# anadodik/sdmm-mitsuba

Measured on AMD Instinct MI355X. Metric: EM samples/sec (NxK resp) at K=128, N=2^20, higher is better.
Workload: dtype f32; 1 GPU; responsibility E-step, synthetic 5D sample batch (configs[1]); K=128, N=1048576, global_batch=1048576, samples_per_gpu=1048576, parallelism=sample-sharded x1 (strong: N fixed), layout=SoA fp32 in, [N][K] fp32 out

## Files before the change

sdmm-mitsuba_amd/csrc/estep_split.hip:

```cpp
#include "sdmm_device.h"

namespace sdmm {

namespace {

typedef float f2 __attribute__((ext_vector_type(2)));
typedef float f4 __attribute__((ext_vector_type(4)));
typedef __bf16 bf8 __attribute__((ext_vector_type(8)));
typedef __bf16 bf2 __attribute__((ext_vector_type(2)));
typedef unsigned u4 __attribute__((ext_vector_type(4)));

template <bool B> struct Tag { static constexpr bool value = B; };

constexpr float kLog2Norm5S = -6.628740082514092f;

__device__ __forceinline__ f2 spl(float x) { return (f2)(x); }
__device__ __forceinline__ f2 pfma(f2 a, f2 b, f2 c) { return __builtin_elementwise_fma(a, b, c); }
__device__ __forceinline__ f2 pmul(f2 a, f2 b) { return a * b; }
__device__ __forceinline__ f2 padd(f2 a, f2 b) { return a + b; }

__device__ __forceinline__ unsigned pk(float lo, float hi) {
    const bf2 v = __builtin_convertvector(f2{lo, hi}, bf2);
    return __builtin_bit_cast(unsigned, v);
}
// ... 375 lines not shown
#pragma unroll
        for (int r = 0; r < R; ++r)
#pragma unroll
            for (int j = 0; j < 4; ++j) {
                pdf[r][j] = P3[j & 1] + D3[j >> 1] + (float)(16 * r + j);
                acc.x += pdf[r][j];
            }
#else
        {
            bf8 F[2][8];
            f4 dp[2];
            frags(0, F[0], dp[0]);
#pragma unroll
            for (int r = 0; r < R; ++r) {
                f4 D[8];
                forms(F[r & 1], Bs, Bd, D);
                __builtin_amdgcn_sched_barrier(0);
                pair_math(r, Tag<false>{}, D, dp[r & 1]);
                if (r + 1 < R) frags(r + 1, F[(r + 1) & 1], dp[(r + 1) & 1]);
                __builtin_amdgcn_sched_barrier(0);
            }
        }
#endif
        const bool odd = cbits > __builtin_bit_cast(uint32_t, -0.9999995f) || !((acc.x + acc.y) + (acc2.x + acc2.y) >= 0.0f);
        if (__builtin_amdgcn_ballot_w64(odd) != 0) {
            bf8 bd2 = Bd, bs2 = Bs;
            asm volatile("" : "+v"(bd2), "+v"(bs2));
            acc = f2{0.0f, 0.0f};
            acc2 = f2{0.0f, 0.0f};
#pragma unroll
            for (int r = 0; r < R; ++r) {
                bf8 F[8];
                f4 dp, D[8];
                frags(r, F, dp);
                forms(F, bs2, bd2, D);
                pair_math(r, Tag<true>{}, D, dp);
            }
        }
        float S = (acc.x + acc.y) + (acc2.x + acc2.y);
        S += __shfl_xor(S, 16);
        S += __shfl_xor(S, 32);
        const float S2 = dif ? fmaf(1.0f - kHeuristicWeight, S, kHeuristicWeight * hp) : S;
        const float inv = __builtin_amdgcn_rcpf(S2);
        const bool fin = __builtin_isfinite(inv) && !dzero;
        gsc_p = fin ? (dif ? inv * (1.0f - kHeuristicWeight) : inv) : 0.0f;
        const bool bad = __builtin_amdgcn_ballot_w64(!__builtin_isfinite(S)) != 0;
        full_p = (t + 16 <= s1) && (16 * R == K) && !bad;
        tp = t;
    }
    flush();
    wait_vm<0>();
}

#ifndef SDMM_SPLIT_R8_WPB
#define SDMM_SPLIT_R8_WPB 12
#define SDMM_SPLIT_R8_OCC 3
#endif
#define SDMM_SPLIT_CONFIGS(X) X(1, 4, 4) X(2, 4, 4) X(4, 4, 4) X(8, SDMM_SPLIT_R8_WPB, SDMM_SPLIT_R8_OCC)

static void split_cfg(int R, int , int* wpb, int* occ) {
    *wpb = 4;
    *occ = 4;
    if (R == 8) {
        *wpb = SDMM_SPLIT_R8_WPB;
        *occ = SDMM_SPLIT_R8_OCC;
    }
}

bool estep_resp_split_supported(int Kp) { return Kp % 16 == 0 && Kp / 16 <= 8 && (Kp / 16 & (Kp / 16 - 1)) == 0; }

hipError_t launch_estep_resp_split(int variant, const float* ep, int Kp, int K, const SamplesDev& s, int64_t n,
                                   int64_t resident_waves, float* resp, hipStream_t st) {
    if (!estep_resp_split_supported(Kp) || K > Kp || resident_waves <= 0) return hipErrorInvalidValue;
    const int R = Kp / 16;
    int wpb, occ;
    split_cfg(R, variant, &wpb, &occ);
    const int64_t tiles = (n + 15) / 16;
    const int64_t blocks = ((tiles < resident_waves ? tiles : resident_waves) + wpb - 1) / wpb;
    const int64_t waves = blocks * wpb;
#define X(RR, WW, OO)                                                                                          \
    if (R == RR && wpb == WW && occ == OO) {                                                                   \
        hipLaunchKernelGGL((estep_resp_split_kernel<RR, WW, OO>), dim3((unsigned)blocks), dim3(64 * WW), 0, st, ep, \
                           Kp, K, s, n, waves, resp);                                                          \
        return hipGetLastError();                                                                              \
    }
    SDMM_SPLIT_CONFIGS(X)
#undef X
    return hipErrorInvalidValue;
}

hipError_t estep_resp_split_occupancy(int variant, int Kp, int* waves_per_cu) {
    const int R = Kp / 16;
    int wpb, occ;
    split_cfg(R, variant, &wpb, &occ);
    int blocks = 0;
#define X(RR, WW, OO)                                                                                          \
    if (R == RR && wpb == WW && occ == OO) {                                                                   \
        hipError_t e = hipOccupancyMaxActiveBlocksPerMultiprocessor(                                           \
            &blocks, reinterpret_cast<const void*>(&estep_resp_split_kernel<RR, WW, OO>), 64 * WW, 0);         \
        *waves_per_cu = blocks * WW;                                                                           \
        return e;                                                                                              \
    }
    SDMM_SPLIT_CONFIGS(X)
#undef X
    return hipErrorInvalidValue;
}

const char* estep_resp_split_name(int variant, int Kp) {
    static thread_local char buf[64];
    int wpb, occ;
    split_cfg(Kp / 16, variant, &wpb, &occ);
    snprintf(buf, sizeof buf, "estep_resp_split_kernel<%d,%d,%d>", Kp / 16, wpb, occ);
    return buf;
}

}
```

sdmm-mitsuba_amd/csrc/sdmm_api.cpp:

```cpp
#include <hip/hip_runtime.h>
#include <rccl/rccl.h>

#include <cmath>
#include <cstdlib>
#include <cstdio>
#include <cstring>
#include <new>
#include <string>
#include <vector>
#include <algorithm>
#include <atomic>
#include <future>
#include <thread>
#include <mutex>

#include "../../include/sdmm_gpu.h"
#include "sdmm_device.h"
#include "render_device.h"
#include "host_xfer.h"

#pragma clang fp contract(off)

namespace sdmm {
hipError_t launch_estep_resp(int cpl, int lps, const float* ep, int Kp, int K, const SamplesDev& s,
// ... 356 lines not shown
        float cov[25] = {0};
        for (int i = 0; i < 5; ++i) cov[6 * i] = 1.0f;
        for (int i = 0; i < 3; ++i)
            for (int j = 0; j < 3; ++j)
                cov[5 * i + j] = (s[i] * s[j] * widthVarSqr + t[i] * t[j] * widthVarSqr) +
                                 n[i] * n[j] * depthVarSqr;
        const float dcov = (float)(2.0 * PI * (double)directionalInit);
        cov[18] = dcov; cov[24] = dcov; cov[19] = 0.0f; cov[23] = 0.0f;
        float bPrior[25] = {0};
        for (int i = 0; i < 5; ++i) bPrior[6 * i] = 1.0f;
        for (int i = 0; i < 3; ++i)
            for (int j = 0; j < 3; ++j)
                bPrior[5 * i + j] = s[i] * s[j] * 1e-4f + t[i] * t[j] * 1e-4f + n[i] * n[j] * 1e-4f;
        bPrior[18] = 1e-5f; bPrior[24] = 1e-5f;
        float theta = 0.0f;
        for (int ti = 0; ti < (int)nThetas; ++ti) {
            float rn = (float)(((double)rng.next_float() - 0.5) * 2e-1);
            theta = (float)((double)theta + (0.5 * PI / (double)(nThetas + 1.0f) + (double)rn));
            const float cosTheta = fl_cos(theta);
            const float sinTheta = std::sqrt(1.0f - cosTheta * cosTheta);
            float phi = 0.0f;
            for (int fi = 0; fi < (int)nPhis; ++fi) {
                rn = (float)(((double)rng.next_float() - 0.5) * 1e-1);
                phi = (float)((double)phi + (2.0 * PI / (double)nPhis + (double)rn));
                const float sinPhi = fl_sin(phi), cosPhi = fl_cos(phi);
                const float dl0 = sinTheta * cosPhi, dl1 = sinTheta * sinPhi, dl2 = cosTheta;
                float* mean = means + 6 * k;
                for (int i = 0; i < 3; ++i) mean[i] = p[i];
                for (int i = 0; i < 3; ++i) mean[3 + i] = (s[i] * dl0 + t[i] * dl1) + n[i] * dl2;
                std::memcpy(covs + 25 * k, cov, sizeof(cov));
                weights[k] = 1.0f / (float)K;
                std::memcpy(bpriors + 25 * k, bPrior, sizeof(bPrior));
                for (int i = 0; i < 3; ++i)
                    for (int j = 0; j < 3; ++j) bdepth[9 * k + 3 * i + j] = n[i] * n[j] * 1e-6f;
                ++k;
            }
        }
    }
}

}

struct Slab {
    void* p = nullptr;
    std::atomic<int> refs{0};
    hipStream_t st = nullptr;
};

struct sdmm_mix {
    int K = 0, Kp = 0, cpl = 1, lps = 64;
    int rcpl = 2, rlps = 64;
    int rtile = 0;
    int rvariant = 4;
    int stile = 0;
    int svariant = 0;
    int device = 0;
    int cus = 256;
    int resp_blocks = 2, stats_blocks = 2;
    int guide_cap = kGuideCapDefault;
    mutable int* guide_fb = nullptr;
    mutable int64_t guide_fb_cap = 0;
    mutable GuideSortScratch guide_sort{};
    mutable ProductScratch product_scratch{};
    int guide_order = 1;
    hipStream_t stream = nullptr;
    hipStream_t own_stream = nullptr;
    sdmm_em_params params{};
    float norm2 = 0, norm3 = 0, norm5 = 0;
    bool initialised = false;

    void* block = nullptr;
    struct Slab* slab = nullptr;
    CanonDev C{};
    EmStateDev S{};
    float* ep = nullptr;
    float* gp = nullptr;
    double* stats = nullptr;
    double* tmp_mean = nullptr;
    double* tmp_cov = nullptr;
    unsigned* mcount = nullptr;
    float* partials = nullptr;
    int partial_rows = 0;
    int pstride = 0;
    void* staging = nullptr;
    size_t staging_bytes = 0;
    void* batch_dev = nullptr;
    void* batch_host = nullptr;
    mutable void* it_dev = nullptr;
    mutable void* it_host = nullptr;
    mutable size_t it_cap = 0;
    size_t batch_bytes = 0;
    hipEvent_t batch_copied = nullptr;
    hipEvent_t batch_done = nullptr;
    double* shard_stats = nullptr;
    size_t shard_bytes = 0;
};

struct sdmm_comm {
    int rank = 0, nranks = 1, device = 0;
    ncclComm_t nccl = nullptr;
    sdmm_host_allreduce_f64 h_allreduce = nullptr;
    sdmm_host_broadcast h_broadcast = nullptr;
    void* user = nullptr;
    void* pinned = nullptr;
    size_t pinned_bytes = 0;
};
// ... 272 lines not shown
        m->gp = gp;
        m->stats = stats;
        m->tmp_mean = tmean;
        m->tmp_cov = tcov;
        m->mcount = mcount;
    }
    return (off + 255) / 256 * 256;
}

void constructor_scalars(const sdmm_mix* m, double* scal) {
    for (int i = 0; i < SC_COUNT; ++i) scal[i] = 0.0;
    scal[SC_NORM] = 1.0;
    scal[SC_ALPHA] = (double)m->params.alpha;
    scal[SC_NI] = (double)m->params.ni_prior_minus_one;
    scal[SC_DECP] = m->params.decrease_prior ? 1.0 : 0.0;
    scal[SC_CUT] = 32.0;
}

struct OccCache {
    int K = -1, kern = -1, resp = 0, stats = 0;
};

int create_impl(int K, const sdmm_em_params* params, int device, hipStream_t ordered, bool on_stream,
                sdmm_mix** out, void* ext_block) {
    if (!out) return fail(SDMM_E_INVALID, "out is NULL");
    *out = nullptr;
    int cpl, lps;
    if (K < 1 || choose_layout(K, cpl, lps)) return fail(SDMM_E_INVALID, "K must be in [1, 512]");
    sdmm_mix* m = new (std::nothrow) sdmm_mix();
    if (!m) return fail(SDMM_E_NOMEM, "out of host memory");
    m->K = K;
    m->cpl = cpl;
    m->lps = lps;
    m->Kp = cpl * lps;
    m->device = device;
    if (params) m->params = *params; else sdmm_em_params_default(&m->params);
    m->norm2 = norm_const(2);
    m->norm3 = norm_const(3);
    m->norm5 = norm_const(5);
    m->pstride = ((ST_FIELDS * m->Kp + 2 + 3) / 4) * 4;

    auto cleanup = [&](int code) { sdmm_destroy(m); return code; };
    if (hipSetDevice(device) != hipSuccess) return cleanup(fail(SDMM_E_HIP, "hipSetDevice failed"));
    (void)hipDeviceGetAttribute(&m->cus, hipDeviceAttributeMultiprocessorCount, device);
    if (m->cus <= 0) m->cus = 256;
    m->rcpl = cpl;
    m->rlps = lps;
    if (K > 64 && K <= 128) { m->rcpl = 4; m->rlps = 32; }
    {
        const char* ev = std::getenv("SDMM_RESP_KERNEL");
        const bool legacy = ev && std::strcmp(ev, "legacy") == 0;
        const bool mfma = ev && std::strcmp(ev, "mfma") == 0;
        const bool tile = ev && std::strcmp(ev, "tile") == 0;
        const bool split = ev && std::strcmp(ev, "split") == 0;
        if (K > 64 && K <= 128 && !legacy && !mfma) {
            m->rtile = 1;
            m->rcpl = 2;
            m->rlps = 64;
            if (!tile && estep_resp_split_supported(m->Kp)) m->rtile = 3;
        }
        if (mfma) m->rtile = 2;
        if (split && estep_resp_split_supported(m->Kp)) m->rtile = 3;
        if (K > 64 && K <= 128) m->stile = 1;
        if (K > 128 && K <= 512) m->stile = 2;
    }
    static thread_local OccCache occ[8];
    OccCache& oc = occ[(K * 7 + device) & 7];
    const int kern = ((m->rtile * 16 + m->rvariant) * 16 + m->stile) * 16 + m->svariant;
    if (oc.K == K * 64 + device && oc.kern == kern) {
        m->resp_blocks = oc.resp;
        m->stats_blocks = oc.stats;
    } else {
        int unused = 0;
        if (estep_occupancy(m->rcpl, m->rlps, m->Kp, &m->resp_blocks, &unused) != hipSuccess ||
            estep_occupancy(m->cpl, m->lps, m->Kp, &unused, &m->stats_blocks) != hipSuccess)
            return cleanup(fail(SDMM_E_HIP, "E-step occupancy query failed"));
        if (m->rtile == 2 && estep_resp_mfma_occupancy(m->rvariant, m->Kp, &m->resp_blocks) != hipSuccess)
            return cleanup(fail(SDMM_E_HIP, "E-step occupancy query failed"));
        if (m->rtile == 3) {
            int wpc = 0;
            if (estep_resp_split_occupancy(m->rvariant, m->Kp, &wpc) != hipSuccess)
                return cleanup(fail(SDMM_E_HIP, "E-step occupancy query failed"));
            m->resp_blocks = wpc;
        }
        if (m->rtile == 1 && estep_resp_tile_occupancy(m->rvariant, &m->resp_blocks) != hipSuccess)
            return cleanup(fail(SDMM_E_HIP, "E-step occupancy query failed"));
        if (m->stile && estep_stats_tile_occupancy(m->svariant, m->Kp, &m->stats_blocks) != hipSuccess)
            return cleanup(fail(SDMM_E_HIP, "E-step occupancy query failed"));
        oc.K = K * 64 + device;
        oc.kern = kern;
        oc.resp = m->resp_blocks;
        oc.stats = m->stats_blocks;
    }
    if (on_stream) {
        m->stream = ordered;
    } else {
        if (hipStreamCreateWithFlags(&m->own_stream, hipStreamNonBlocking) != hipSuccess)
            return cleanup(fail(SDMM_E_HIP, "hipStreamCreate failed"));
        m->stream = m->own_stream;
    }

    if (ext_block) {
        layout_block(m, (char*)ext_block);
        *out = m;
        return SDMM_OK;
    }
    const size_t total = layout_block(m, nullptr);
    if (hipMalloc(&m->block, total) != hipSuccess) return cleanup(fail(SDMM_E_HIP, "hipMalloc failed"));
    if (hipMemsetAsync(m->block, 0, total, m->stream) != hipSuccess)
        return cleanup(fail(SDMM_E_HIP, "hipMemsetAsync failed"));
    layout_block(m, (char*)m->block);
    const size_t Kc = (size_t)K;
    double* sc = m->S.scalars;
    float* bp = m->S.bPriors;
    float* bd = m->S.bDepth;
    double scal[SC_COUNT];
    constructor_scalars(m, scal);
    (void)Kc;
    const float eps = (float)m->params.epsilon;
    if (launch_init_state(K, scal, m->params.bprior, eps, sc, bp, bd, m->stream) != hipSuccess)
        return cleanup(fail(SDMM_E_HIP, "state init kernel launch failed"));
    if (launch_pack_all(K, m->Kp, m->C, m->ep, m->gp, m->norm5, m->stream) != hipSuccess)
        return cleanup(fail(SDMM_E_HIP, "pack kernel launch failed"));
    if (!on_stream && hipStreamSynchronize(m->stream) != hipSuccess)
        return cleanup(fail(SDMM_E_HIP, "hipStreamSynchronize failed"));
    *out = m;
    return SDMM_OK;
}

int create_many(int K, const sdmm_em_params* params, int device, hipStream_t st, int n, sdmm_mix** out) {
    if (n < 0 || (n > 0 && !out)) return fail(SDMM_E_INVALID, "invalid argument");
    for (int i = 0; i < n; ++i) out[i] = nullptr;
    if (n == 0) return SDMM_OK;
    if (hipSetDevice(device) != hipSuccess) return fail(SDMM_E_HIP, "hipSetDevice failed");
// ... 172 lines not shown
    if (n < 0 || (n > 0 && (!src || !dst))) return fail(SDMM_E_INVALID, "invalid argument");
    if (n == 0) return SDMM_OK;
    int r = check_same_kind(src, n);
    if (!r) r = check_same_kind(dst, n);
    if (r) return r;
    if (src[0]->K != dst[0]->K || src[0]->device != dst[0]->device)
        return fail(SDMM_E_INVALID, "sources and destinations must share K and device");
    HIP_TRY(hipSetDevice(dst[0]->device));
    const hipStream_t st = dst[0]->stream;
    for (int i = 1; i < n; ++i)
        if (dst[i]->stream != st) HIP_TRY(hipStreamSynchronize(dst[i]->stream));
    return copy_prefix_many(src, dst, n, st);
}

int sdmm_num_components(const sdmm_mix* m) { return m ? m->K : 0; }

int sdmm_set_guide_order(sdmm_mix* m, int coherent) {
    if (!m) return fail(SDMM_E_INVALID, "null handle");
    m->guide_order = coherent ? 1 : 0;
    return SDMM_OK;
}

int sdmm_set_guide_capacity(sdmm_mix* m, int cap) {
    if (!m) return fail(SDMM_E_INVALID, "null handle");
    if (cap < 0 || cap > kGuideCapMax) return fail(SDMM_E_INVALID, "guide capacity must be in [0, 64]");
    m->guide_cap = cap;
    return SDMM_OK;
}

int sdmm_guide_fallback_count(const sdmm_mix* m, int* count) {
    if (!m || !count) return fail(SDMM_E_INVALID, "invalid argument");
    *count = 0;
    if (!m->guide_fb) return SDMM_OK;
    HIP_TRY(hipSetDevice(m->device));
    HIP_TRY(hipMemcpyAsync(count, m->guide_fb, sizeof(int), hipMemcpyDeviceToHost, m->stream));
    HIP_TRY(hipStreamSynchronize(m->stream));
    return SDMM_OK;
}

int sdmm_layout(const sdmm_mix* m, int* resp_cpl, int* resp_lps, int* stats_cpl, int* stats_lps) {
    if (!m) return fail(SDMM_E_INVALID, "null handle");
    if (resp_cpl) *resp_cpl = m->rcpl;
    if (resp_lps) *resp_lps = m->rlps;
    if (stats_cpl) *stats_cpl = m->cpl;
    if (stats_lps) *stats_lps = m->lps;
    return SDMM_OK;
}

const char* sdmm_kernel_name(const sdmm_mix* m, int which) {
    if (!m) return "";
    static thread_local char buf[64];
    if (which == 0) {
        if (m->rtile == 3) {
            std::snprintf(buf, sizeof buf, "%s", estep_resp_split_name(m->rvariant, m->Kp));
            return buf;
        } else if (m->rtile == 2) {
            std::snprintf(buf, sizeof buf, "%s", estep_resp_mfma_name(m->rvariant, m->Kp));
            return buf;
        } else if (m->rtile) {
            std::snprintf(buf, sizeof buf, "%s", estep_resp_tile_name(m->rvariant));
            return buf;
        }
        std::snprintf(buf, sizeof buf, "estep_resp_kernel<%d,%d>", m->rcpl, m->rlps);
        return buf;
    }
    if (m->stile == 2)
        std::snprintf(buf, sizeof buf, "estep_stats_tile_kernel<%d,2,true>", m->Kp / 128);
    else if (m->stile)
        std::snprintf(buf, sizeof buf, "estep_stats_tile_kernel<4,%d>", m->svariant == 1 ? 3 : 2);
    else
        std::snprintf(buf, sizeof buf, "estep_stats_kernel<%d,%d>", m->cpl, m->lps);
    return buf;
}

int sdmm_set_stream(sdmm_mix* m, void* hip_stream) {
    if (!m) return fail(SDMM_E_INVALID, "handle is NULL");
    HIP_TRY(hipSetDevice(m->device));
    if ((hipStream_t)hip_stream != m->stream) HIP_TRY(hipStreamSynchronize(m->stream));
    m->stream = (hipStream_t)hip_stream;
    return SDMM_OK;
}

void* sdmm_get_stream(const sdmm_mix* m) { return m ? (void*)m->stream : nullptr; }

int sdmm_synchronize(sdmm_mix* m) {
    if (!m) return fail(SDMM_E_INVALID, "handle is NULL");
    HIP_TRY(hipSetDevice(m->device));
    HIP_TRY(hipStreamSynchronize(m->stream));
    return SDMM_OK;
}

int sdmm_hemisphere_init_host(const float* positions, const float* normals, int n_pos, float depth_prior,
                              float min_spatial_distance, uint64_t seed, float* weights, float* means,
                              float* covs, float* bpriors, float* bdepth) {
    if (!positions || !normals || n_pos <= 0 || !weights || !means || !covs || !bpriors || !bdepth)
        return fail(SDMM_E_INVALID, "invalid argument to sdmm_hemisphere_init_host");
    hemisphere_init(positions, normals, n_pos, depth_prior, min_spatial_distance, seed, weights, means,
                    covs, bpriors, bdepth);
    return SDMM_OK;
}

static int upload_and_set(sdmm_mix* m, const float* weights, const float* means, const float* covs) {
    const size_t K = (size_t)m->K;
    char* pin = nullptr;
    HIP_TRY(bounce_buf(8 * 31 * K + 4 * K, &pin));
    double* md = (double*)pin;
    double* cd = md + 6 * K;
// ... 606 lines not shown
    r = stage_host_samples(m0, s, &d);
    if (r) return r;
    r = sdmm_em_step_batched(mixes, n_mix, &d, seg, iterations);
    const hipError_t e = hipStreamSynchronize(m0->stream);
    if (r) return r;
    if (e != hipSuccess) return fail(SDMM_E_HIP, std::string("sdmm_em_step_batched_host: ") + hipGetErrorString(e));
    return SDMM_OK;
}

int sdmm_em_step_batched_host_iters(sdmm_mix* const* mixes, int n_mix, const sdmm_samples* s, const int64_t* seg,
                                    const int* iterations) {
    if (n_mix < 0 || (n_mix > 0 && (!mixes || !mixes[0] || !iterations))) return fail(SDMM_E_INVALID, "invalid argument");
    if (n_mix == 0) return SDMM_OK;
    int r = check_samples(s);
    if (r) return r;
    if (s->n == 0) return sdmm_em_step_batched_iters(mixes, n_mix, s, seg, iterations);
    sdmm_mix* m0 = mixes[0];
    HIP_TRY(hipSetDevice(m0->device));
    sdmm_samples d;
    r = stage_host_samples(m0, s, &d);
    if (r) return r;
    r = sdmm_em_step_batched_iters(mixes, n_mix, &d, seg, iterations);
    const hipError_t e = hipStreamSynchronize(m0->stream);
    if (r) return r;
    if (e != hipSuccess) return fail(SDMM_E_HIP, std::string("sdmm_em_step_batched_host: ") + hipGetErrorString(e));
    return SDMM_OK;
}

int sdmm_em_step_host(sdmm_mix* m, const sdmm_samples* s, int iterations) {
    if (!m) return fail(SDMM_E_INVALID, "handle is NULL");
    HIP_TRY(hipSetDevice(m->device));
    int r = check_samples(s);
    if (r) return r;
    if (s->n == 0) return SDMM_OK;
    if (!m->initialised) return fail(SDMM_E_STATE, "mixture not initialised");
    sdmm_samples d;
    r = stage_host_samples(m, s, &d);
    if (r) return r;
    r = sdmm_em_step(m, &d, iterations);
    const hipError_t e = hipStreamSynchronize(m->stream);
    if (r) return r;
    if (e != hipSuccess) return fail(SDMM_E_HIP, std::string("sdmm_em_step_host: ") + hipGetErrorString(e));
    return SDMM_OK;
}

int sdmm_responsibilities(sdmm_mix* m, const sdmm_samples* s, float* resp) {
    if (!m || !resp) return fail(SDMM_E_INVALID, "invalid argument");
    if (!m->initialised) return fail(SDMM_E_STATE, "mixture not initialised");
    HIP_TRY(hipSetDevice(m->device));
    int r = check_samples(s);
    if (r) return r;
    if (s->n == 0) return SDMM_OK;
    if (m->rtile == 3) {
        const int64_t resident = (int64_t)m->cus * (m->resp_blocks > 0 ? m->resp_blocks : 1);
        HIP_TRY(launch_estep_resp_split(m->rvariant, m->ep, m->Kp, m->K, to_dev(s), s->n, resident, resp, m->stream));
        return SDMM_OK;
    }
    if (m->rtile == 2) {
        const int64_t resident = (int64_t)m->cus * 4 * (m->resp_blocks > 0 ? m->resp_blocks : 1);
        int64_t chunk = (s->n + 3 * resident - 1) / (3 * resident);
        chunk = ((chunk + 15) / 16) * 16;
        if (chunk < 64) chunk = 64;
        HIP_TRY(launch_estep_resp_mfma(m->rvariant, m->ep, m->Kp, m->K, to_dev(s), s->n, chunk, resp, m->stream));
        return SDMM_OK;
    }
    if (m->rtile) {
        const int64_t resident = (int64_t)m->cus * 4 * (m->resp_blocks > 0 ? m->resp_blocks : 1);
        int64_t chunk = (s->n + 3 * resident - 1) / (3 * resident);
        chunk = ((chunk + 63) / 64) * 64;
        if (chunk < 64) chunk = 64;
        HIP_TRY(launch_estep_resp_tile(m->rvariant, m->ep, m->Kp, m->K, to_dev(s), s->n, chunk, resp, m->stream));
        return SDMM_OK;
    }
    const Split sp = split_for(m, s->n, m->rlps, m->resp_blocks);
    HIP_TRY(launch_estep_resp(m->rcpl, m->rlps, m->ep, m->Kp, m->K, to_dev(s), s->n, sp.chunk, resp,
                              m->stream));
    return SDMM_OK;
}

int sdmm_guide_batch(const sdmm_mix* m, int64_t nq, const float* const c[3], const float* const u[3],
                     float* const d[3], float* pdf, int32_t* comp) {
    if (!m || !c || !u || !d || !pdf || !comp) return fail(SDMM_E_INVALID, "invalid argument");
    if (!m->initialised) return fail(SDMM_E_STATE, "mixture not initialised");
    HIP_TRY(hipSetDevice(m->device));
    if (nq <= 0) return SDMM_OK;
    int r = ensure_guide_scratch(m, nq);
    if (r) return r;
    HIP_TRY(launch_guide(m->gp, m->Kp, m->K, nq, c, u, nullptr, d, pdf, comp, m->norm2, m->norm3,
                         m->guide_cap, m->guide_fb, m->guide_fb + 1, m->cus, m->stream, guide_order(m, nq),
                         (int*)m->guide_sort.keys[0]));
    return SDMM_OK;
}

int sdmm_pdf_batch(const sdmm_mix* m, int64_t nq, const float* const c[3], const float* const d[3],
                   float* pdf) {
    if (!m || !c || !d || !pdf) return fail(SDMM_E_INVALID, "invalid argument");
    if (!m->initialised) return fail(SDMM_E_STATE, "mixture not initialised");
    HIP_TRY(hipSetDevice(m->device));
    if (nq <= 0) return SDMM_OK;
    int r = ensure_guide_scratch(m, nq);
    if (r) return r;
    HIP_TRY(launch_guide(m->gp, m->Kp, m->K, nq, c, nullptr, d, nullptr, pdf, nullptr, m->norm2, m->norm3,
                         m->guide_cap, m->guide_fb, m->guide_fb + 1, m->cus, m->stream, guide_order(m, nq),
                         (int*)m->guide_sort.keys[0]));
    return SDMM_OK;
}

static int check_bsdf(const sdmm_bsdf_table* b, const int32_t* material, const float* const frame[9]) {
// ... 1412 lines not shown
```

Baseline: 6.915 billion samples/s.

## Add split-pairs E-step kernel with deferred rare-tile recompute path

Adds a new split responsibility kernel that runs a fast non-rare pdf path per tile. Tiles whose values look out of range are recorded in a small per-wave LDS list and recomputed afterwards with the careful (rare) math. It also adds an optional two-tile-per-fragment-read mode with interleaved MFMA scheduling, and env knobs for the variant and wave count. By default the single-tile variant of the new kernel replaces the old split kernel for K=128. The aim is to drop the cost of slow-path handling from the common loop, at the price of extra LDS, more code, and a serial recompute pass when rare tiles appear.

```diff
diff --git a/sdmm-mitsuba_amd/csrc/estep_split.hip b/sdmm-mitsuba_amd/csrc/estep_split.hip
--- a/sdmm-mitsuba_amd/csrc/estep_split.hip
+++ b/sdmm-mitsuba_amd/csrc/estep_split.hip
@@ -451,19 +451,398 @@
     wait_vm<0>();
 }
 
-#ifndef SDMM_SPLIT_R8_WPB
-#define SDMM_SPLIT_R8_WPB 12
-#define SDMM_SPLIT_R8_OCC 3
+#ifndef SDMM_SPLIT_PAIR_IL
+#define SDMM_SPLIT_PAIR_IL 0
 #endif
-#define SDMM_SPLIT_CONFIGS(X) X(1, 4, 4) X(2, 4, 4) X(4, 4, 4) X(8, SDMM_SPLIT_R8_WPB, SDMM_SPLIT_R8_OCC)
-
-static void split_cfg(int R, int , int* wpb, int* occ) {
-    *wpb = 4;
-    *occ = 4;
-    if (R == 8) {
-        *wpb = SDMM_SPLIT_R8_WPB;
-        *occ = SDMM_SPLIT_R8_OCC;
-    }
+constexpr int kPairAhead = 1;
+constexpr int kRareCap = 16;
+
+template <int V> struct Int { static constexpr int value = V; };
+
+template <int T, int AH, int R, int KK = 0>
+__device__ __forceinline__ void read_feat_window(int k, unsigned addr, f4& a, f4& b) {
+    constexpr int N = 2 * T * AH + T * R * KK;
+    if constexpr (KK == AH + 1) {
+        read_feat<N>(addr, a, b);
+    } else {
+        if (k == KK) read_feat<N>(addr, a, b);
+        else read_feat_window<T, AH, R, KK + 1>(k, addr, a, b);
+    }
+}
+
+template <int R, int WPB, int OCC, int T, bool BAL>
+__global__ void __launch_bounds__(64 * WPB, OCC)
+estep_resp_split_pairs_kernel(const float* __restrict__ ep, int Kp, int K, SamplesDev s, int64_t n, int64_t nwaves,
+                        float* __restrict__ resp) {
+    static_assert(T == 1 || T == 2, "one tile or a pair per fragment read");
+    constexpr int AH = T == 2 ? kPairAhead : kFeatAhead;
+    constexpr int SLOTS = AH + 1, SLOT_U4 = T * kFeatSlotU4;
+    static_assert(2 * T * AH + T * R * (AH + 1) <= 63, "the counted wait exceeds the six bits of vmcnt");
+    constexpr int NC = R * 8 * 64, ND = R * 4, NS = R == 8 ? 16 * 16 : 0, NF = SLOTS * SLOT_U4, NL = kRareCap / 4;
+    constexpr int NTOT = WPB * NF + NC + ND + WPB * NS + WPB * NL;
+    static_assert(NTOT * 16 <= 163840, "the carved LDS block exceeds the 160 KB of a CU");
+    static_assert(WPB * NF * 16 <= 65536, "LDS-DMA destinations stay below 64 KB");
+    __shared__ u4 smem[NTOT];
+    const int wid = __builtin_amdgcn_readfirstlane(threadIdx.x >> 6);
+    u4* const ring = smem + wid * NF;
+    u4* const cimg = smem + WPB * NF;
+    f4* const dimg = (f4*)(cimg + NC);
+    f4* const st = (f4*)(cimg + NC + ND + wid * NS);
+    int* const lst = (int*)(cimg + NC + ND + WPB * NS + wid * NL);
+
+    const float o_scene[3] = {kOrigin, kOrigin, kOrigin};
+    for (int idx = threadIdx.x; idx < NC; idx += 64 * WPB)
+        cimg[idx] = coef_frag(ep, Kp, idx >> 9, (idx >> 6) & 7, idx & 63, o_scene);
+    for (int i = threadIdx.x; i < ND; i += 64 * WPB) {
+        const float* d = ep + EP_DIPI * Kp + 4 * i;
+        dimg[i] = f4{d[0], d[1], d[2], d[3]};
+    }
+    __syncthreads();
+
+    const int lane = threadIdx.x & 63;
+    const int64_t wave = BAL ? (int64_t)wid * gridDim.x + blockIdx.x : (int64_t)blockIdx.x * WPB + wid;
+    const int64_t s0 = 16 * wave, step = 16 * nwaves, s1 = n;
+    if (wave >= nwaves || s0 >= n) return;
+
+    const int g = lane >> 4;
+    const int col = lane & 15;
+    const bool has_h = s.hpdf != nullptr, has_d = s.isDiffuse != nullptr;
+
+    const int pl = lane & 3, sl = lane >> 2;
+    const uintptr_t src0 = (uintptr_t)(pl == 0 ? s.x[0] : pl == 1 ? s.x[1] : pl == 2 ? s.x[2] : s.x[3]);
+    const bool byteplane = pl == 3 && has_d;
+    const uintptr_t src1 = (uintptr_t)(pl == 0   ? s.x[4]
+                                       : pl == 1 ? s.x[5]
+                                       : pl == 2 ? (has_h ? s.hpdf : s.x[0])
+                                                 : (has_d ? (const float*)s.isDiffuse : s.x[0]));
+    const int sh1 = byteplane ? 0 : 2;
+    const unsigned ring_lds = (unsigned)(uintptr_t)(__attribute__((address_space(3))) u4*)ring;
+    auto dma_iter = [&](int i) __attribute__((always_inline)) {
+#pragma unroll
+        for (int j = 0; j < T; ++j) {
+            int64_t smp = s0 + (int64_t)(T * i + j) * step + sl;
+            smp = (smp < s1) ? smp : s1 - 1;
+            const uintptr_t a0 = src0 + ((uintptr_t)smp << 2);
+            const uintptr_t a1 = (src1 + ((uintptr_t)smp << sh1)) & ~(uintptr_t)3;
+            dma_pair(a0, a1, ring_lds + (unsigned)((i % SLOTS) * SLOT_U4 + j * kFeatSlotU4) * 16u);
+        }
+    };
+
+    auto frags = [&](int r, bf8 (&F)[8], f4& dp) __attribute__((always_inline)) {
+#pragma unroll
+        for (int f = 0; f < 8; ++f) F[f] = __builtin_bit_cast(bf8, cimg[(r * 8 + f) * 64 + lane]);
+        dp = dimg[r * 4 + g];
+    };
+    auto forms = [&](const bf8 (&F)[8], bf8 bs, bf8 bd, f4 (&D)[8]) __attribute__((always_inline)) {
+        const f4 z = f4{0.0f, 0.0f, 0.0f, 0.0f};
+#pragma unroll
+        for (int f = 0; f < 8; ++f) D[f] = __builtin_amdgcn_mfma_f32_16x16x32_bf16(F[f], f < 3 ? bd : bs, z, 0, 0, 0);
+    };
+
+    struct TileIn {
+        bf8 Bs, Bd;
+        bool dzero, dif;
+        float hp;
+    };
+    auto decode = [&](const float (&P3)[3], const float (&D3)[3], bool dif, float hp) __attribute__((always_inline)) {
+        TileIn in;
+        in.dzero = D3[0] == 0.0f && D3[1] == 0.0f && D3[2] == 0.0f;
+        in.dif = dif;
+        in.hp = hp;
+        in.Bd = a_frag(D3, g, false);
+        const float x[3] = {P3[0] - kOrigin, P3[1] - kOrigin, P3[2] - kOrigin};
+        in.Bs = a_frag(x, g, true);
+        return in;
+    };
+
+    float pdf[T][R][4];
+    float gsc_p[T];
+    bool full_p[T];
+    int64_t tp[T];
+#pragma unroll
+    for (int j = 0; j < T; ++j) {
+        gsc_p[j] = 0.0f;
+        full_p[j] = false;
+        tp[j] = -1;
+    }
+    auto flush_tile = [&](auto jc) __attribute__((always_inline)) {
+        constexpr int j = decltype(jc)::value;
+        if (tp[j] < 0) return;
+        const int64_t t = tp[j];
+        const float gs = gsc_p[j];
+        tp[j] = -1;
+        if (kDiagNoStore && gs != -1.0f) return;
+        float* row = resp + (t + col) * (int64_t)K + 4 * g;
+        if (full_p[j] && R != 8) {
+#pragma unroll
+            for (int r = 0; r < R; ++r)
+                __builtin_nontemporal_store(f4{pdf[j][r][0], pdf[j][r][1], pdf[j][r][2], pdf[j][r][3]},
+                                            (f4*)(row + 16 * r));
+        } else if (full_p[j]) {
+#pragma unroll
+            for (int h = 0; h < 2; ++h) {
+#pragma unroll
+                for (int rr = 0; rr < 4; ++rr) {
+                    const int r = (4 * h + rr) % R;
+                    st[col * 16 + ((4 * rr + g) ^ col)] = f4{pdf[j][r][0], pdf[j][r][1], pdf[j][r][2], pdf[j][r][3]};
+                }
+                __builtin_amdgcn_wave_barrier();
+#pragma unroll
+                for (int i = 0; i < 4; ++i) {
+                    const int rw = g + 4 * i, ch = col;
+                    const f4 v = st[rw * 16 + (ch ^ rw)];
+                    __builtin_nontemporal_store(v, (f4*)(resp + (t + rw) * (int64_t)K + 64 * h + 4 * ch));
+                }
+                __builtin_amdgcn_wave_barrier();
+            }
+        } else if (t + col < s1) {
+#pragma unroll
+            for (int r = 0; r < R; ++r)
+#pragma unroll
+                for (int jj = 0; jj < 4; ++jj) {
+                    const float o = gs != 0.0f ? pdf[j][r][jj] : 0.0f;
+                    if (16 * r + 4 * g + jj < K) __builtin_nontemporal_store(o, row + 16 * r + jj);
+                }
+        }
+    };
+    auto flush_all = [&]() __attribute__((always_inline)) {
+        flush_tile(Int<0>{});
+        if constexpr (T == 2) flush_tile(Int<1>{});
+    };
+
+    auto pair_math = [&](auto jc, int r, auto rare, const f4 (&D)[8], const f4& dp, f2& acc, f2& acc2,
+                         uint32_t& cbits) __attribute__((always_inline)) {
+        constexpr int j = decltype(jc)::value;
+        constexpr bool RARE = decltype(rare)::value;
+        if constexpr (!RARE)
+            cbits = __builtin_elementwise_max(
+                cbits, __builtin_elementwise_max(__builtin_elementwise_max(fbits(D[0][0]), fbits(D[0][1])),
+                                                 __builtin_elementwise_max(fbits(D[0][2]), fbits(D[0][3]))));
+        f2 p[2];
+        pdf_quad<RARE>(D[0], D[1], D[2], D[3], D[4], D[5], D[6], D[7], dp, p);
+        pdf[j][r][0] = p[0].x;
+        pdf[j][r][1] = p[0].y;
+        pdf[j][r][2] = p[1].x;
+        pdf[j][r][3] = p[1].y;
+        acc = padd(acc, p[0]);
+        acc2 = padd(acc2, p[1]);
+    };
+    auto normalise = [&](auto jc, int64_t t, const TileIn& in, f2 acc, f2 acc2) __attribute__((always_inline)) {
+        constexpr int j = decltype(jc)::value;
+        float S = (acc.x + acc.y) + (acc2.x + acc2.y);
+        S += __shfl_xor(S, 16);
+        S += __shfl_xor(S, 32);
+        const float S2 = in.dif ? fmaf(1.0f - kHeuristicWeight, S, kHeuristicWeight * in.hp) : S;
+        const float inv = __builtin_amdgcn_rcpf(S2);
+        const bool fin = __builtin_isfinite(inv) && !in.dzero;
+        gsc_p[j] = fin ? (in.dif ? inv * (1.0f - kHeuristicWeight) : inv) : 0.0f;
+        const bool bad = __builtin_amdgcn_ballot_w64(!__builtin_isfinite(S)) != 0;
+        full_p[j] = (t + 16 <= s1) && (16 * R == K) && !bad;
+        tp[j] = t;
+#pragma unroll
+        for (int r = 0; r < R; ++r) {
+            const f2 lo = f2{pdf[j][r][0], pdf[j][r][1]} * spl(gsc_p[j]);
+            const f2 hi = f2{pdf[j][r][2], pdf[j][r][3]} * spl(gsc_p[j]);
+            pdf[j][r][0] = lo.x;
+            pdf[j][r][1] = lo.y;
+            pdf[j][r][2] = hi.x;
+            pdf[j][r][3] = hi.y;
+        }
+    };
+
+    int cnt = 0;
+    auto is_rare = [&](f2 acc, f2 acc2, uint32_t cbits) __attribute__((always_inline)) {
+        const bool odd =
+            cbits > __builtin_bit_cast(uint32_t, -0.9999995f) || !((acc.x + acc.y) + (acc2.x + acc2.y) >= 0.0f);
+        return __builtin_amdgcn_ballot_w64(odd) != 0;
+    };
+    auto finish = [&](auto jc, bool rare, int q, int64_t t, const TileIn& in, f2 acc, f2 acc2)
+                      __attribute__((always_inline)) {
+        constexpr int j = decltype(jc)::value;
+        if (rare) {
+            lst[cnt] = q;
+            ++cnt;
+            full_p[j] = false;
+            tp[j] = -1;
+            return;
+        }
+        normalise(jc, t, in, acc, acc2);
+    };
+
+    auto ring_tile = [&](int k, bool window_full, unsigned addr, int64_t t) __attribute__((always_inline)) {
+        f4 fa, fb;
+        if (kDiagNoStore) read_feat<2 * T * AH>(addr, fa, fb);
+        else if (!window_full) read_feat<0>(addr, fa, fb);
+        else read_feat_window<T, AH, R>(k, addr, fa, fb);
+        const float P3[3] = {fa.x, fa.y, fa.z};
+        const float D3[3] = {fa.w, fb.x, fb.y};
+        const int64_t ic = (t + col < s1) ? t + col : s1 - 1;
+        const bool dif = has_d && ((fbits(fb.w) >> (8 * (int)((uintptr_t)(s.isDiffuse + ic) & 3))) & 0xffu) != 0u;
+        return decode(P3, D3, dif, has_h ? fb.z : 0.0f);
+    };
+
+    int it = 0;
+    for (;;) {
+        const int it0 = it;
+#pragma unroll
+        for (int a = 0; a < AH; ++a) dma_iter(it0 + a);
+        unsigned hist = 0;
+        bool more = false;
+        for (;; ++it) {
+            const int64_t tA = s0 + (int64_t)(T * it) * step;
+            if (tA >= s1) break;
+            if (cnt + T > kRareCap) {
+                more = true;
+                break;
+            }
+            dma_iter(it + AH);
+            bool stored_full = tp[0] >= 0 && full_p[0];
+            if constexpr (T == 2) stored_full = stored_full && tp[1] >= 0 && full_p[1];
+            hist = (hist << 1) | (stored_full ? 1u : 0u);
+            flush_all();
+            const int k = it - it0 < AH + 1 ? it - it0 : AH + 1;
+            const unsigned need = (1u << k) - 1u;
+            const bool window_full = (hist & need) == need;
+            const unsigned slot_lds = ring_lds + (unsigned)((it % SLOTS) * SLOT_U4) * 16u + 16u * col;
+            const int64_t tB = tA + step;
+            if (T == 2 && tB < s1) {
+                const TileIn inA = ring_tile(k, window_full, slot_lds, tA);
+                const TileIn inB = ring_tile(k, window_full, slot_lds + kFeatSlotU4 * 16u, tB);
+                f2 accA = f2{0.0f, 0.0f}, acc2A = f2{0.0f, 0.0f}, accB = f2{0.0f, 0.0f}, acc2B = f2{0.0f, 0.0f};
+                uint32_t cbA = 0, cbB = 0;
+#if SDMM_SPLIT_PAIR_IL
+                bf8 F[8];
+                f4 dp[2], DA[8], DB[8];
+                frags(0, F, dp[0]);
+                forms(F, inA.Bs, inA.Bd, DA);
+                __builtin_amdgcn_sched_barrier(0);
+#pragma unroll
+                for (int r = 0; r < R; ++r) {
+                    forms(F, inB.Bs, inB.Bd, DB);
+                    pair_math(Int<0>{}, r, Tag<false>{}, DA, dp[r & 1], accA, acc2A, cbA);
+#pragma unroll
+                    for (int i = 0; i < 8; ++i) {
+                        __builtin_amdgcn_sched_group_barrier(0x008, 1, 0);
+                        __builtin_amdgcn_sched_group_barrier(0x002, SDMM_SPLIT_PAIR_IL, 0);
+                    }
+                    __builtin_amdgcn_sched_barrier(0);
+                    if (r + 1 < R) {
+                        frags(r + 1, F, dp[(r + 1) & 1]);
+                        forms(F, inA.Bs, inA.Bd, DA);
+                    }
+                    pair_math(Int<T - 1>{}, r, Tag<false>{}, DB, dp[r & 1], accB, acc2B, cbB);
+                    if (r + 1 < R) {
+                        __builtin_amdgcn_sched_group_barrier(0x100, 9, 0);
+                        __builtin_amdgcn_sched_group_barrier(0x002, 12, 0);
+#pragma unroll
+                        for (int i = 0; i < 8; ++i) {
+                            __builtin_amdgcn_sched_group_barrier(0x008, 1, 0);
+                            __builtin_amdgcn_sched_group_barrier(0x002, SDMM_SPLIT_PAIR_IL - 1, 0);
+                        }
+                    }
+                    __builtin_amdgcn_sched_barrier(0);
+                }
+#else
+                bf8 F[8];
+                f4 dp[2];
+                frags(0, F, dp[0]);
+#pragma unroll
+                for (int r = 0; r < R; ++r) {
+                    f4 D[8];
+                    forms(F, inA.Bs, inA.Bd, D);
+                    __builtin_amdgcn_sched_barrier(0);
+                    pair_math(Int<0>{}, r, Tag<false>{}, D, dp[r & 1], accA, acc2A, cbA);
+                    __builtin_amdgcn_sched_barrier(0);
+                    forms(F, inB.Bs, inB.Bd, D);
+                    __builtin_amdgcn_sched_barrier(0);
+                    if (r + 1 < R) frags(r + 1, F, dp[(r + 1) & 1]);
+                    pair_math(Int<T - 1>{}, r, Tag<false>{}, D, dp[r & 1], accB, acc2B, cbB);
+                    __builtin_amdgcn_sched_barrier(0);
+                }
+#endif
+                const bool rareA = is_rare(accA, acc2A, cbA), rareB = is_rare(accB, acc2B, cbB);
+                finish(Int<0>{}, rareA, T * it, tA, inA, accA, acc2A);
+                finish(Int<T - 1>{}, rareB, T * it + 1, tB, inB, accB, acc2B);
+            } else {
+                const TileIn in = ring_tile(k, window_full, slot_lds, tA);
+                f2 acc = f2{0.0f, 0.0f}, acc2 = f2{0.0f, 0.0f};
+                uint32_t cb = 0;
+                bf8 F[2][8];
+                f4 dp[2];
+                frags(0, F[0], dp[0]);
+#pragma unroll
+                for (int r = 0; r < R; ++r) {
+                    f4 D[8];
+                    forms(F[r & 1], in.Bs, in.Bd, D);
+                    __builtin_amdgcn_sched_barrier(0);
+                    pair_math(Int<0>{}, r, Tag<false>{}, D, dp[r & 1], acc, acc2, cb);
+                    if (r + 1 < R) frags(r + 1, F[(r + 1) & 1], dp[(r + 1) & 1]);
+                    __builtin_amdgcn_sched_barrier(0);
+                }
+                finish(Int<0>{}, is_rare(acc, acc2, cb), T * it, tA, in, acc, acc2);
+            }
+        }
+        flush_all();
+        wait_vm<0>();
+        for (int e = 0; e < cnt; ++e) {
+            asm volatile("" ::: "memory");
+            const int q = __builtin_amdgcn_readfirstlane(lst[e]);
+            const int64_t t = s0 + (int64_t)q * step;
+            const int64_t ic = (t + col < s1) ? t + col : s1 - 1;
+            const float P3[3] = {s.x[0][ic], s.x[1][ic], s.x[2][ic]};
+            const float D3[3] = {s.x[3][ic], s.x[4][ic], s.x[5][ic]};
+            const TileIn in = decode(P3, D3, has_d && s.isDiffuse[ic] != 0, has_h ? s.hpdf[ic] : 0.0f);
+            f2 acc = f2{0.0f, 0.0f}, acc2 = f2{0.0f, 0.0f};
+            uint32_t cb = 0;
+#pragma unroll
+            for (int r = 0; r < R; ++r) {
+                bf8 F[8];
+                f4 dp, D[8];
+                frags(r, F, dp);
+                forms(F, in.Bs, in.Bd, D);
+                pair_math(Int<0>{}, r, Tag<true>{}, D, dp, acc, acc2, cb);
+            }
+            normalise(Int<0>{}, t, in, acc, acc2);
+            flush_tile(Int<0>{});
+        }
+        cnt = 0;
+        if (!more) break;
+    }
+}
+
+#ifndef SDMM_SPLIT_PAIR_WPB
+#define SDMM_SPLIT_PAIR_WPB 8
+#define SDMM_SPLIT_PAIR_OCC 2
+#endif
+#ifndef SDMM_SPLIT_BAL
+#define SDMM_SPLIT_BAL 0
+#endif
+constexpr bool kSplitBal = SDMM_SPLIT_BAL != 0;
+
+struct SplitCfg {
+    int wpb, occ, tiles;
+};
+using SplitKernel = void (*)(const float*, int, int, SamplesDev, int64_t, int64_t, float*);
+
+static SplitCfg split_cfg(int R, int variant) {
+    if (variant == 1) return R == 8 ? SplitCfg{12, 3, 0} : SplitCfg{4, 4, 0};
+    if (variant == 2 && R == 8) return SplitCfg{SDMM_SPLIT_PAIR_WPB, SDMM_SPLIT_PAIR_OCC, 2};
+    return R == 8 ? SplitCfg{12, 3, 1} : SplitCfg{4, 4, 1};
+}
+static SplitKernel split_kernel(int R, const SplitCfg& c) {
+    if (c.tiles == 0) {
+        if (R == 1) return estep_resp_split_kernel<1, 4, 4>;
+        if (R == 2) return estep_resp_split_kernel<2, 4, 4>;
+        if (R == 4) return estep_resp_split_kernel<4, 4, 4>;
+        if (R == 8) return estep_resp_split_kernel<8, 12, 3>;
+        return nullptr;
+    }
+    if (R == 1) return estep_resp_split_pairs_kernel<1, 4, 4, 1, kSplitBal>;
+    if (R == 2) return estep_resp_split_pairs_kernel<2, 4, 4, 1, kSplitBal>;
+    if (R == 4) return estep_resp_split_pairs_kernel<4, 4, 4, 1, kSplitBal>;
+    if (R == 8 && c.tiles == 1) return estep_resp_split_pairs_kernel<8, 12, 3, 1, kSplitBal>;
+    if (R == 8) return estep_resp_split_pairs_kernel<8, SDMM_SPLIT_PAIR_WPB, SDMM_SPLIT_PAIR_OCC, 2, kSplitBal>;
+    return nullptr;
 }
 
 bool estep_resp_split_supported(int Kp) { return Kp % 16 == 0 && Kp / 16 <= 8 && (Kp / 16 & (Kp / 16 - 1)) == 0; }
@@ -472,44 +851,34 @@
                                    int64_t resident_waves, float* resp, hipStream_t st) {
     if (!estep_resp_split_supported(Kp) || K > Kp || resident_waves <= 0) return hipErrorInvalidValue;
     const int R = Kp / 16;
-    int wpb, occ;
-    split_cfg(R, variant, &wpb, &occ);
+    const SplitCfg c = split_cfg(R, variant);
+    const SplitKernel kern = split_kernel(R, c);
+    if (!kern) return hipErrorInvalidValue;
     const int64_t tiles = (n + 15) / 16;
-    const int64_t blocks = ((tiles < resident_waves ? tiles : resident_waves) + wpb - 1) / wpb;
-    const int64_t waves = blocks * wpb;
-#define X(RR, WW, OO)                                                                                          \
-    if (R == RR && wpb == WW && occ == OO) {                                                                   \
-        hipLaunchKernelGGL((estep_resp_split_kernel<RR, WW, OO>), dim3((unsigned)blocks), dim3(64 * WW), 0, st, ep, \
-                           Kp, K, s, n, waves, resp);                                                          \
-        return hipGetLastError();                                                                              \
-    }
-    SDMM_SPLIT_CONFIGS(X)
-#undef X
-    return hipErrorInvalidValue;
+    const int64_t blocks = ((tiles < resident_waves ? tiles : resident_waves) + c.wpb - 1) / c.wpb;
+    const int64_t waves = blocks * c.wpb;
+    hipLaunchKernelGGL(kern, dim3((unsigned)blocks), dim3(64 * c.wpb), 0, st, ep, Kp, K, s, n, waves, resp);
+    return hipGetLastError();
 }
 
 hipError_t estep_resp_split_occupancy(int variant, int Kp, int* waves_per_cu) {
     const int R = Kp / 16;
-    int wpb, occ;
-    split_cfg(R, variant, &wpb, &occ);
+    const SplitCfg c = split_cfg(R, variant);
+    const SplitKernel kern = split_kernel(R, c);
+    if (!kern) return hipErrorInvalidValue;
     int blocks = 0;
-#define X(RR, WW, OO)                                                                                          \
-    if (R == RR && wpb == WW && occ == OO) {                                                                   \
-        hipError_t e = hipOccupancyMaxActiveBlocksPerMultiprocessor(                                           \
-            &blocks, reinterpret_cast<const void*>(&estep_resp_split_kernel<RR, WW, OO>), 64 * WW, 0);         \
-        *waves_per_cu = blocks * WW;                                                                           \
-        return e;                                                                                              \
-    }
-    SDMM_SPLIT_CONFIGS(X)
-#undef X
-    return hipErrorInvalidValue;
+    hipError_t e =
+        hipOccupancyMaxActiveBlocksPerMultiprocessor(&blocks, reinterpret_cast<const void*>(kern), 64 * c.wpb, 0);
+    *waves_per_cu = blocks * c.wpb;
+    return e;
 }
 
 const char* estep_resp_split_name(int variant, int Kp) {
     static thread_local char buf[64];
-    int wpb, occ;
-    split_cfg(Kp / 16, variant, &wpb, &occ);
-    snprintf(buf, sizeof buf, "estep_resp_split_kernel<%d,%d,%d>", Kp / 16, wpb, occ);
+    const SplitCfg c = split_cfg(Kp / 16, variant);
+    if (c.tiles == 0) snprintf(buf, sizeof buf, "estep_resp_split_kernel<%d,%d,%d>", Kp / 16, c.wpb, c.occ);
+    else snprintf(buf, sizeof buf, "estep_resp_split_pairs_kernel<%d,%d,%d,%d,%s>", Kp / 16, c.wpb, c.occ, c.tiles,
+                  kSplitBal ? "true" : "false");
     return buf;
 }
 
diff --git a/sdmm-mitsuba_amd/csrc/sdmm_api.cpp b/sdmm-mitsuba_amd/csrc/sdmm_api.cpp
--- a/sdmm-mitsuba_amd/csrc/sdmm_api.cpp
+++ b/sdmm-mitsuba_amd/csrc/sdmm_api.cpp
@@ -432,6 +432,8 @@
     int rcpl = 2, rlps = 64;
     int rtile = 0;
     int rvariant = 4;
+    int rsplit = 0;
+    int64_t resp_waves = 0;
     int stile = 0;
     int svariant = 0;
     int device = 0;
@@ -810,7 +812,11 @@
         const bool legacy = ev && std::strcmp(ev, "legacy") == 0;
         const bool mfma = ev && std::strcmp(ev, "mfma") == 0;
         const bool tile = ev && std::strcmp(ev, "tile") == 0;
-        const bool split = ev && std::strcmp(ev, "split") == 0;
+        const bool split1 = ev && std::strcmp(ev, "split1") == 0;
+        const bool split2 = ev && std::strcmp(ev, "split2") == 0;
+        const bool split = split1 || split2 || (ev && std::strcmp(ev, "split") == 0);
+        m->rsplit = split1 ? 1 : (split2 ? 2 : 0);
+        if (const char* wv = std::getenv("SDMM_RESP_WAVES")) m->resp_waves = std::atoll(wv);
         if (K > 64 && K <= 128 && !legacy && !mfma) {
             m->rtile = 1;
             m->rcpl = 2;
@@ -824,7 +830,7 @@
     }
     static thread_local OccCache occ[8];
     OccCache& oc = occ[(K * 7 + device) & 7];
-    const int kern = ((m->rtile * 16 + m->rvariant) * 16 + m->stile) * 16 + m->svariant;
+    const int kern = (((m->rtile * 16 + m->rvariant) * 16 + m->stile) * 16 + m->svariant) * 4 + m->rsplit;
     if (oc.K == K * 64 + device && oc.kern == kern) {
         m->resp_blocks = oc.resp;
         m->stats_blocks = oc.stats;
@@ -837,7 +843,7 @@
             return cleanup(fail(SDMM_E_HIP, "E-step occupancy query failed"));
         if (m->rtile == 3) {
             int wpc = 0;
-            if (estep_resp_split_occupancy(m->rvariant, m->Kp, &wpc) != hipSuccess)
+            if (estep_resp_split_occupancy(m->rsplit, m->Kp, &wpc) != hipSuccess)
                 return cleanup(fail(SDMM_E_HIP, "E-step occupancy query failed"));
             m->resp_blocks = wpc;
         }
@@ -1116,7 +1122,7 @@
     static thread_local char buf[64];
     if (which == 0) {
         if (m->rtile == 3) {
-            std::snprintf(buf, sizeof buf, "%s", estep_resp_split_name(m->rvariant, m->Kp));
+            std::snprintf(buf, sizeof buf, "%s", estep_resp_split_name(m->rsplit, m->Kp));
             return buf;
         } else if (m->rtile == 2) {
             std::snprintf(buf, sizeof buf, "%s", estep_resp_mfma_name(m->rvariant, m->Kp));
@@ -1829,8 +1835,9 @@
     if (r) return r;
     if (s->n == 0) return SDMM_OK;
     if (m->rtile == 3) {
-        const int64_t resident = (int64_t)m->cus * (m->resp_blocks > 0 ? m->resp_blocks : 1);
-        HIP_TRY(launch_estep_resp_split(m->rvariant, m->ep, m->Kp, m->K, to_dev(s), s->n, resident, resp, m->stream));
+        int64_t resident = (int64_t)m->cus * (m->resp_blocks > 0 ? m->resp_blocks : 1);
+        if (m->resp_waves > 0 && m->resp_waves < resident) resident = m->resp_waves;
+        HIP_TRY(launch_estep_resp_split(m->rsplit, m->ep, m->Kp, m->K, to_dev(s), s->n, resident, resp, m->stream));
         return SDMM_OK;
     }
     if (m->rtile == 2) {
```

After: 6.906 billion samples/s (median of 2 runs). No clear change (-0.1%).
